# LuoweiZhou/VLP

Hardware: NVIDIA H100
Metric: image_text_samples_per_sec (higher is better)
Workload: dtype bf16

## Files before the change

### vlp_b200/csrc/common.cuh

```cuda
#pragma once
#include <cuda.h>
#include <cuda_bf16.h>
#include <cuda_runtime.h>
#include <stdint.h>

#include "wgmma.cuh"

namespace vlpk {

__device__ __forceinline__ uint32_t smem_u32(const void* p) {
  return static_cast<uint32_t>(__cvta_generic_to_shared(p));
}

__device__ __forceinline__ uint32_t lane_id() { return threadIdx.x & 31u; }

__device__ __forceinline__ bool elect_one() {
  uint32_t pred = 0;
  asm volatile(
      "{\n\t"
      ".reg .pred P;\n\t"
      "elect.sync _|P, 0xffffffff;\n\t"
      "selp.u32 %0, 1, 0, P;\n\t"
      "}\n"
      : "=r"(pred));
  return pred != 0;
}

__device__ __forceinline__ void mbar_init(uint64_t* bar, uint32_t count) {
  asm volatile("mbarrier.init.shared::cta.b64 [%0], %1;" ::"r"(smem_u32(bar)), "r"(count) : "memory");
}
__device__ __forceinline__ void fence_mbar_init() {
  asm volatile("fence.mbarrier_init.release.cluster;" ::: "memory");
}
__device__ __forceinline__ void fence_proxy_async_smem() {
  asm volatile("fence.proxy.async.shared::cta;" ::: "memory");
}
__device__ __forceinline__ void mbar_arrive_expect_tx(uint64_t* bar, uint32_t bytes) {
  asm volatile("mbarrier.arrive.expect_tx.shared::cta.b64 _, [%0], %1;" ::"r"(smem_u32(bar)), "r"(bytes)
               : "memory");
}
__device__ __forceinline__ void mbar_arrive(uint64_t* bar) {
  asm volatile("mbarrier.arrive.shared::cta.b64 _, [%0];" ::"r"(smem_u32(bar)) : "memory");
}
__device__ __forceinline__ bool mbar_try_wait(uint64_t* bar, uint32_t parity) {
  uint32_t ok;
  asm volatile(
      "{\n\t"
      ".reg .pred P;\n\t"
      "mbarrier.try_wait.parity.shared::cta.b64 P, [%1], %2;\n\t"
      "selp.u32 %0, 1, 0, P;\n\t"
      "}\n"
      : "=r"(ok)
      : "r"(smem_u32(bar)), "r"(parity)
      : "memory");
  return ok != 0;
}
__device__ __forceinline__ void mbar_wait(uint64_t* bar, uint32_t parity) {
  uint32_t spins = 0;
  while (!mbar_try_wait(bar, parity)) {
    if (++spins > (1u << 28)) { __trap(); }
  }
}

__device__ __forceinline__ void pdl_launch_dependents() { asm volatile("griddepcontrol.launch_dependents;" ::: "memory"); }
__device__ __forceinline__ void pdl_wait() { asm volatile("griddepcontrol.wait;" ::: "memory"); }

__device__ __forceinline__ void tma_prefetch_desc(const CUtensorMap* m) {
  asm volatile("prefetch.tensormap [%0];" ::"l"(reinterpret_cast<uint64_t>(m)) : "memory");
}
__device__ __forceinline__ void tma_load_2d(void* dst, const CUtensorMap* m, uint64_t* bar, int c0, int c1) {
  asm volatile(
      "cp.async.bulk.tensor.2d.shared::cluster.global.tile.mbarrier::complete_tx::bytes [%0], [%1, {%3, %4}], [%2];"
      ::"r"(smem_u32(dst)), "l"(reinterpret_cast<uint64_t>(m)), "r"(smem_u32(bar)), "r"(c0), "r"(c1)
      : "memory");
}
__device__ __forceinline__ void tma_load_3d(void* dst, const CUtensorMap* m, uint64_t* bar, int c0, int c1,
                                            int c2) {
  asm volatile(
      "cp.async.bulk.tensor.3d.shared::cluster.global.tile.mbarrier::complete_tx::bytes [%0], [%1, {%3, %4, %5}], "
      "[%2];" ::"r"(smem_u32(dst)),
      "l"(reinterpret_cast<uint64_t>(m)), "r"(smem_u32(bar)), "r"(c0), "r"(c1), "r"(c2)
      : "memory");
}
__device__ __forceinline__ void tma_store_2d(const CUtensorMap* m, const void* src, int c0, int c1) {
  asm volatile("cp.async.bulk.tensor.2d.global.shared::cta.tile.bulk_group [%0, {%2, %3}], [%1];" ::"l"(
                   reinterpret_cast<uint64_t>(m)),
               "r"(smem_u32(src)), "r"(c0), "r"(c1)
               : "memory");
}
__device__ __forceinline__ void tma_store_3d(const CUtensorMap* m, const void* src, int c0, int c1, int c2) {
  asm volatile("cp.async.bulk.tensor.3d.global.shared::cta.tile.bulk_group [%0, {%2, %3, %4}], [%1];" ::"l"(
                   reinterpret_cast<uint64_t>(m)),
               "r"(smem_u32(src)), "r"(c0), "r"(c1), "r"(c2)
               : "memory");
}
__device__ __forceinline__ void tma_reduce_add_2d(const CUtensorMap* m, const void* src, int c0, int c1) {
  asm volatile("cp.reduce.async.bulk.tensor.2d.global.shared::cta.add.tile.bulk_group [%0, {%2, %3}], [%1];" ::"l"(
                   reinterpret_cast<uint64_t>(m)),
               "r"(smem_u32(src)), "r"(c0), "r"(c1)
               : "memory");
}
__device__ __forceinline__ void tma_reduce_add_3d(const CUtensorMap* m, const void* src, int c0, int c1, int c2) {
  asm volatile("cp.reduce.async.bulk.tensor.3d.global.shared::cta.add.tile.bulk_group [%0, {%2, %3, %4}], [%1];" ::"l"(
                   reinterpret_cast<uint64_t>(m)),
               "r"(smem_u32(src)), "r"(c0), "r"(c1), "r"(c2)
               : "memory");
}
__device__ __forceinline__ void tma_store_commit() { asm volatile("cp.async.bulk.commit_group;" ::: "memory"); }
template <int N>
__device__ __forceinline__ void tma_store_wait_read() {
  asm volatile("cp.async.bulk.wait_group.read %0;" ::"n"(N) : "memory");
}
template <int N>
__device__ __forceinline__ void tma_store_wait() {
  asm volatile("cp.async.bulk.wait_group %0;" ::"n"(N) : "memory");
}

__device__ __forceinline__ void wgmma_fence() { asm volatile("wgmma.fence.sync.aligned;" ::: "memory"); }
__device__ __forceinline__ void wgmma_commit() { asm volatile("wgmma.commit_group.sync.aligned;" ::: "memory"); }
template <int N>
__device__ __forceinline__ void wgmma_wait() {
  asm volatile("wgmma.wait_group.sync.aligned %0;" ::"n"(N) : "memory");
}
template <int N>
__device__ __forceinline__ void reg_fence(float (&d)[N]) {
#pragma unroll
  for (int i = 0; i < N; ++i) asm volatile("" : "+f"(d[i])::"memory");
}

__device__ __forceinline__ uint64_t wgmma_desc_sw128(uint32_t saddr, uint32_t lbo_bytes, uint32_t sbo_bytes) {
  uint64_t d = 0;
  d |= static_cast<uint64_t>((saddr & 0x3FFFFu) >> 4);
  d |= static_cast<uint64_t>((lbo_bytes >> 4) & 0x3FFFu) << 16;
  d |= static_cast<uint64_t>((sbo_bytes >> 4) & 0x3FFFu) << 32;
  d |= 1ull << 62;
  return d;
}

__device__ __forceinline__ uint32_t pack_bf16x2(float lo, float hi) {
  __nv_bfloat162 v = __floats2bfloat162_rn(lo, hi);
  return *reinterpret_cast<uint32_t*>(&v);
}
__device__ __forceinline__ float2 unpack_bf16x2(uint32_t u) {
  __nv_bfloat162 v = *reinterpret_cast<__nv_bfloat162*>(&u);
  return __bfloat1622float2(v);
}
__device__ __forceinline__ float bf16_round(float x) { return __bfloat162float(__float2bfloat16_rn(x)); }

__device__ __forceinline__ float fast_ex2(float x) {
  float y;
  asm("ex2.approx.ftz.f32 %0, %1;" : "=f"(y) : "f"(x));
  return y;
}
__device__ __forceinline__ float fast_rcp(float x) {
  float y;
  asm("rcp.approx.ftz.f32 %0, %1;" : "=f"(y) : "f"(x));
  return y;
}

__device__ __forceinline__ void gelu_and_grad(float x, float& g, float& d) {
  const float ax = fabsf(x);
  const float e = fast_ex2(-0.72134752044448170f * x * x);
  const float t = fast_rcp(fmaf(0.3275911f * 0.70710678118654752f, ax, 1.0f));
  float poly = fmaf(1.061405429f, t, -1.453152027f);
  poly = fmaf(poly, t, 1.421413741f);
  poly = fmaf(poly, t, -0.284496736f);
  poly = fmaf(poly, t, 0.254829592f);
  poly *= t;
  const float erf_abs = fmaf(-poly, e, 1.0f);
  const float cdf = 0.5f * (1.0f + copysignf(erf_abs, x));
  g = x * cdf;
  d = fmaf(x * 0.3989422804014327f, e, cdf);
}

struct Philox {
  __device__ __forceinline__ static uint4 gen(uint64_t seed, uint64_t ctr_hi, uint64_t ctr_lo) {
    uint32_t k0 = static_cast<uint32_t>(seed), k1 = static_cast<uint32_t>(seed >> 32);
    uint4 c = make_uint4(static_cast<uint32_t>(ctr_lo), static_cast<uint32_t>(ctr_lo >> 32),
                         static_cast<uint32_t>(ctr_hi), static_cast<uint32_t>(ctr_hi >> 32));
#pragma unroll
    for (int i = 0; i < 10; ++i) {
      const uint32_t hi0 = __umulhi(0xD2511F53u, c.x), lo0 = 0xD2511F53u * c.x;
      const uint32_t hi1 = __umulhi(0xCD9E8D57u, c.z), lo1 = 0xCD9E8D57u * c.z;
      c = make_uint4(hi1 ^ c.y ^ k0, lo1, hi0 ^ c.w ^ k1, lo0);
      k0 += 0x9E3779B9u;
      k1 += 0xBB67AE85u;
    }
    return c;
  }
};
__device__ __forceinline__ uint32_t dropout_keep8(uint64_t seed, uint64_t site, uint64_t idx8, uint32_t thresh16) {
  const uint4 r = Philox::gen(seed, site, idx8);
  uint32_t m = 0;
  m |= ((r.x & 0xFFFFu) >= thresh16) ? 1u : 0u;
  m |= ((r.x >> 16) >= thresh16) ? 2u : 0u;
  m |= ((r.y & 0xFFFFu) >= thresh16) ? 4u : 0u;
  m |= ((r.y >> 16) >= thresh16) ? 8u : 0u;
  m |= ((r.z & 0xFFFFu) >= thresh16) ? 16u : 0u;
  m |= ((r.z >> 16) >= thresh16) ? 32u : 0u;
  m |= ((r.w & 0xFFFFu) >= thresh16) ? 64u : 0u;
  m |= ((r.w >> 16) >= thresh16) ? 128u : 0u;
  return m;
}

struct DropoutCfg {
  float p;
  float scale;
  uint32_t thresh16;
  uint64_t seed;
  uint64_t site;
  const unsigned long long* seed_ptr;
  const unsigned char* bits;
};

__device__ __forceinline__ uint64_t drop_seed(const DropoutCfg& d) {
  return (d.p > 0.f && d.seed_ptr != nullptr) ? d.seed + *d.seed_ptr : d.seed;
}

__host__ inline DropoutCfg make_dropout(float p, uint64_t seed, uint64_t site,
                                        const unsigned long long* seed_ptr = nullptr) {
  DropoutCfg d;
  d.bits = nullptr;
  d.seed_ptr = seed_ptr;
  d.p = p;
  d.scale = p > 0.f ? 1.0f / (1.0f - p) : 1.0f;
  d.thresh16 = static_cast<uint32_t>(p * 65536.0f);
  d.seed = seed;
  d.site = site;
  return d;
}

}
```

### vlp_b200/csrc/gemm.cu

```cuda
#include "gemm.cuh"

#include <cstdlib>

#include "host.cuh"

namespace vlpk {

static constexpr int BM = 128;
static constexpr int BK = 64;
static constexpr int NUM_THREADS = 288;
static constexpr int STG_BYTES = 64 * 128;
static constexpr int SMEM_MAX = 232448;
static constexpr int BN = 128;

struct GemmTmaps {
  CUtensorMap a;
  CUtensorMap b[3];
  CUtensorMap d0;
  CUtensorMap d1;
};

struct GemmArgs {
  int M, N, K;
  int b_seg_rows;
  int splits;
  int split_slices;
  const __nv_bfloat16* bias[3];
  const __nv_bfloat16* aux;
  long long ld_aux;
  float relu_scale;
  DropoutCfg drop;
  float* colsum;
};

template <int STAGES>
struct SmemLayout {
  static constexpr int A_BYTES = BM * BK * 2;
  static constexpr int B_BYTES = BN * BK * 2;
  static constexpr int STAGE_BYTES = A_BYTES + B_BYTES;
  static constexpr int OFF_STG = STAGES * STAGE_BYTES;
  static constexpr int OFF_BAR = OFF_STG + 4 * STG_BYTES;
  static constexpr int NUM_BARS = 2 * STAGES;
  static constexpr int TOTAL = OFF_BAR + NUM_BARS * 8;
  static constexpr int DYN_BYTES = TOTAL + 1024;
  static_assert(DYN_BYTES <= SMEM_MAX, "shared memory budget exceeded");
};

struct StageCount {
  static constexpr int value = (SMEM_MAX - 1024 - 4 * STG_BYTES - 256) / (BM * BK * 2 + BN * BK * 2);
};

__device__ __forceinline__ void wg_bar_sync(int cw) {
  asm volatile("bar.sync %0, 128;" ::"r"(cw + 1) : "memory");
}

template <bool A_MN, bool B_MN, int EPI>
__global__ void __launch_bounds__(NUM_THREADS, 1)
gemm_kernel(const __grid_constant__ GemmTmaps tm, const GemmArgs args) {
  constexpr int STAGES = StageCount::value;
  using L = SmemLayout<STAGES>;
  extern __shared__ uint8_t smem_raw[];
  uint8_t* smem = reinterpret_cast<uint8_t*>((reinterpret_cast<uintptr_t>(smem_raw) + 1023) & ~uintptr_t(1023));

  uint64_t* bars = reinterpret_cast<uint64_t*>(smem + L::OFF_BAR);
  uint64_t* full_bar = bars;
  uint64_t* empty_bar = bars + STAGES;

  pdl_launch_dependents();
  const int wg = threadIdx.x >> 7;
  const int lane = threadIdx.x & 31;

  const int num_m = (args.M + BM - 1) / BM;
  const int num_n = (args.N + BN - 1) / BN;
  const int total_kb = (args.K + BK - 1) / BK;
  const int kb_per = (total_kb + args.splits - 1) / args.splits;
  const int num_work = num_m * num_n * args.splits;

  if (threadIdx.x == 0) {
    tma_prefetch_desc(&tm.a);
    tma_prefetch_desc(&tm.b[0]);
    tma_prefetch_desc(&tm.d0);
    for (int i = 0; i < STAGES; ++i) {
      mbar_init(&full_bar[i], 1);
      mbar_init(&empty_bar[i], 8);
    }
    fence_mbar_init();
  }
  __syncthreads();
  pdl_wait();

  if (wg == 2) {
    {
      int stage = 0;
      uint32_t phase = 0;
      for (int w = blockIdx.x; w < num_work; w += gridDim.x) {
        const int n_blk = w % num_n;
        const int m_blk = (w / num_n) % num_m;
        const int split = w / (num_n * num_m);
        const int kb0 = split * kb_per;
        const int kb1 = min(total_kb, kb0 + kb_per);
        const int m0 = m_blk * BM;
        for (int kb = kb0; kb < kb1; ++kb) {
          mbar_wait(&empty_bar[stage], phase ^ 1u);
          if (elect_one()) {
            uint8_t* sA = smem + stage * L::STAGE_BYTES;
            uint8_t* sB = sA + L::A_BYTES;
            mbar_arrive_expect_tx(&full_bar[stage], L::STAGE_BYTES);
            if (!A_MN) {
              tma_load_2d(sA, &tm.a, &full_bar[stage], kb * BK, m0);
            } else {
#pragma unroll
              for (int j = 0; j < BM / 64; ++j) tma_load_2d(sA + j * 8192, &tm.a, &full_bar[stage], m0 + j * 64, kb * BK);
            }
            if (!B_MN) {
              const int n0 = n_blk * BN;
              const int seg = n0 / args.b_seg_rows;
              tma_load_2d(sB, &tm.b[seg], &full_bar[stage], kb * BK, n0 - seg * args.b_seg_rows);
            } else {
              const int k0 = kb * BK;
              const int seg = k0 / args.b_seg_rows;
#pragma unroll
              for (int j = 0; j < BN / 64; ++j)
                tma_load_2d(sB + j * 8192, &tm.b[seg], &full_bar[stage], n_blk * BN + j * 64, k0 - seg * args.b_seg_rows);
            }
          }
          __syncwarp();
          if (++stage == STAGES) {
            stage = 0;
            phase ^= 1u;
          }
        }
      }
    }
  } else {
    const int cw = wg;
    const int t = threadIdx.x - 128 * wg;
    const int fr = (t >> 5) * 16 + (lane >> 2);
    const int fc = (lane & 3) * 2;
    const bool store_thread = (t == 0);
    const uint64_t dseed = drop_seed(args.drop);
    constexpr bool HAS_BIAS = !B_MN && (EPI == EPI_STORE || EPI == EPI_GELU || EPI == EPI_RELU);
    uint8_t* stg0 = smem + L::OFF_STG + cw * 2 * STG_BYTES;
    uint8_t* stg1 = stg0 + STG_BYTES;
    const uint32_t a_base = smem_u32(smem) + cw * 8192;
    const uint32_t b_base = smem_u32(smem) + L::A_BYTES;
    int stage = 0;
    uint32_t phase = 0;
    uint32_t box_seq = 0;
    float acc[BN / 2];
    for (int w = blockIdx.x; w < num_work; w += gridDim.x) {
      const int n_blk = w % num_n;
      const int m_blk = (w / num_n) % num_m;
      const int split = w / (num_n * num_m);
      const int kb0 = split * kb_per;
      const int kb1 = min(total_kb, kb0 + kb_per);
      const int n0 = n_blk * BN;
      const int m0 = m_blk * BM + cw * 64;

      for (int kb = kb0; kb < kb1; ++kb) {
        mbar_wait(&full_bar[stage], phase);
        const uint32_t sa = a_base + stage * L::STAGE_BYTES;
        const uint32_t sb = b_base + stage * L::STAGE_BYTES;
        reg_fence(acc);
        wgmma_fence();
#pragma unroll
        for (int k = 0; k < BK / 16; ++k) {
          const uint64_t adesc = A_MN ? wgmma_desc_sw128(sa + k * 2048, 8192, 1024) : wgmma_desc_sw128(sa + k * 32, 16, 1024);
          const uint64_t bdesc = B_MN ? wgmma_desc_sw128(sb + k * 2048, 8192, 1024) : wgmma_desc_sw128(sb + k * 32, 16, 1024);
          wgmma_m64n128k16_ss<A_MN ? 1 : 0, B_MN ? 1 : 0>(acc, adesc, bdesc, (kb > kb0 || k > 0) ? 1u : 0u);
        }
        wgmma_commit();
        wgmma_wait<0>();
        reg_fence(acc);
        if (lane == 0) mbar_arrive(&empty_bar[stage]);
        if (++stage == STAGES) {
          stage = 0;
          phase ^= 1u;
        }
      }

      if (EPI == EPI_REDUCE_F32) {
        constexpr int NBOX = BN / 32;
#pragma unroll
        for (int c = 0; c < NBOX; ++c) {
          uint8_t* stg = (box_seq & 1u) ? stg1 : stg0;
          if (store_thread) tma_store_wait_read<1>();
          wg_bar_sync(cw);
#pragma unroll
          for (int j = 0; j < 8; ++j) {
            const int i = c * 16 + 2 * j;
            const int r = fr + 8 * (j & 1), col = 8 * (j >> 1) + fc;
            *reinterpret_cast<float2*>(stg + r * 128 + (((col >> 2) ^ (r & 7)) << 4) + (col & 3) * 4) = make_float2(acc[i], acc[i + 1]);
          }
          fence_proxy_async_smem();
          wg_bar_sync(cw);
          if (store_thread) {
            tma_reduce_add_3d(&tm.d0, stg, n0 + c * 32, m0, args.split_slices ? split : 0);
            tma_store_commit();
          }
          ++box_seq;
        }
      } else {
        constexpr int NBOX = BN / 64;
        const __nv_bfloat16* bp = nullptr;
        int bias_off = 0;
        if (HAS_BIAS) {
          const int seg = n0 / args.b_seg_rows;
          bp = args.bias[seg];
          bias_off = seg * args.b_seg_rows;
        }
#pragma unroll
        for (int c = 0; c < NBOX; ++c) {
          uint8_t* stg = (EPI == EPI_GELU) ? stg0 : ((box_seq & 1u) ? stg1 : stg0);
          if (store_thread) {
            if (EPI == EPI_GELU) tma_store_wait_read<0>(); else tma_store_wait_read<1>();
          }
          wg_bar_sync(cw);
#pragma unroll
          for (int j = 0; j < 16; ++j) {
            const int i = c * 32 + 2 * j;
            const int r = fr + 8 * (j & 1), col = 8 * (j >> 1) + fc;
            const int n = n0 + c * 64 + col;
            const long long m = m0 + r;
            float v0 = acc[i], v1 = acc[i + 1];
            if (HAS_BIAS) {
              if (bp != nullptr && n < args.N) {
                const float2 bb = unpack_bf16x2(__ldg(reinterpret_cast<const unsigned int*>(bp + n - bias_off)));
                v0 += bb.x;
                v1 += bb.y;
              }
            }
            const int so = r * 128 + (((col >> 3) ^ (r & 7)) << 4) + (col & 7) * 2;
            if (EPI == EPI_GELU) {
              float g0, d0, g1, d1;
              gelu_and_grad(v0, g0, d0);
              gelu_and_grad(v1, g1, d1);
              *reinterpret_cast<uint32_t*>(stg0 + so) = pack_bf16x2(d0, d1);
              *reinterpret_cast<uint32_t*>(stg1 + so) = pack_bf16x2(g0, g1);
              continue;
            }
            if (EPI == EPI_RELU) {
              uint32_t keep = 0xFFu;
              if (args.drop.p > 0.f)
                keep = dropout_keep8(dseed, args.drop.site, (static_cast<uint64_t>(m) * args.N + (n - fc)) >> 3, args.drop.thresh16);
              v0 = fmaxf(v0, 0.f);
              v1 = fmaxf(v1, 0.f);
              v0 = ((keep >> fc) & 1u) ? v0 * args.drop.scale : 0.f;
              v1 = ((keep >> (fc + 1)) & 1u) ? v1 * args.drop.scale : 0.f;
            } else if (EPI == EPI_ADD || EPI == EPI_MUL || EPI == EPI_DRELU) {
              float2 x = make_float2(0.f, 0.f);
              if (m < args.M && n < args.N) x = unpack_bf16x2(__ldg(reinterpret_cast<const unsigned int*>(args.aux + m * args.ld_aux + n)));
              if (EPI == EPI_ADD) {
                v0 += x.x;
                v1 += x.y;
              } else if (EPI == EPI_MUL) {
                v0 *= x.x;
                v1 *= x.y;
              } else {
                v0 = x.x > 0.f ? v0 * args.relu_scale : 0.f;
                v1 = x.y > 0.f ? v1 * args.relu_scale : 0.f;
              }
            }
            *reinterpret_cast<uint32_t*>(stg + so) = pack_bf16x2(v0, v1);
          }
          fence_proxy_async_smem();
          wg_bar_sync(cw);
          if (store_thread) {
            tma_store_2d(&tm.d0, stg, n0 + c * 64, m0);
            if (EPI == EPI_GELU) tma_store_2d(&tm.d1, stg1, n0 + c * 64, m0);
            tma_store_commit();
          }
          if (EPI != EPI_GELU && args.colsum != nullptr) {
            const int col = t & 63, r0 = (t >> 6) * 32;
            float acc_c = 0.f;
#pragma unroll 8
            for (int rr = r0; rr < r0 + 32; ++rr) {
              const __nv_bfloat16 v = *reinterpret_cast<const __nv_bfloat16*>(stg + rr * 128 + (((col >> 3) ^ (rr & 7)) << 4) + (col & 7) * 2);
              acc_c += __bfloat162float(v);
            }
            if (n0 + c * 64 + col < args.N) atomicAdd(args.colsum + n0 + c * 64 + col, acc_c);
          }
          ++box_seq;
        }
      }
    }
    if (store_thread) tma_store_wait<0>();
  }
}

template <bool A_MN, bool B_MN, int EPI>
static int launch_inst(const GemmTmaps& tm, const GemmArgs& args, int num_work, cudaStream_t stream) {
  constexpr int STAGES = StageCount::value;
  using L = SmemLayout<STAGES>;
  auto kfn = gemm_kernel<A_MN, B_MN, EPI>;
  static bool attr_set = false;
  if (!attr_set) {
    VLPK_CUDA(cudaFuncSetAttribute(kfn, cudaFuncAttributeMaxDynamicSharedMemorySize, L::DYN_BYTES));
    attr_set = true;
  }
  const int max_ctas = gemm_sms();
  const int ctas = num_work < max_ctas ? num_work : max_ctas;
  LaunchScope scope(A_MN ? CAT_GEMM_WGRAD : (B_MN ? CAT_GEMM_DGRAD : CAT_GEMM_FWD), 2.0 * args.M * args.N * args.K, stream);
  VLPK_CUDA(launch_ex(kfn, dim3(ctas), dim3(NUM_THREADS), L::DYN_BYTES, stream, 1, tm, args));
  return 0;
}

static int dispatch(const GemmDesc& g, const GemmTmaps& tm, const GemmArgs& args, int num_work, cudaStream_t s) {
  if (!g.a_mn && !g.b_mn) {
    switch (g.epi) {
      case EPI_STORE: return launch_inst<false, false, EPI_STORE>(tm, args, num_work, s);
      case EPI_GELU: return launch_inst<false, false, EPI_GELU>(tm, args, num_work, s);
      case EPI_RELU: return launch_inst<false, false, EPI_RELU>(tm, args, num_work, s);
      default: break;
    }
  } else if (!g.a_mn && g.b_mn) {
    switch (g.epi) {
      case EPI_STORE: return launch_inst<false, true, EPI_STORE>(tm, args, num_work, s);
      case EPI_ADD: return launch_inst<false, true, EPI_ADD>(tm, args, num_work, s);
      case EPI_MUL: return launch_inst<false, true, EPI_MUL>(tm, args, num_work, s);
      case EPI_DRELU: return launch_inst<false, true, EPI_DRELU>(tm, args, num_work, s);
      case EPI_REDUCE_F32: return launch_inst<false, true, EPI_REDUCE_F32>(tm, args, num_work, s);
      default: break;
    }
  } else if (g.a_mn && g.b_mn) {
    if (g.epi == EPI_REDUCE_F32) return launch_inst<true, true, EPI_REDUCE_F32>(tm, args, num_work, s);
    if (g.epi == EPI_STORE) return launch_inst<true, true, EPI_STORE>(tm, args, num_work, s);
  }
  set_error("gemm: unsupported (a_mn=%d, b_mn=%d, epi=%d) combination", (int)g.a_mn, (int)g.b_mn, g.epi);
  return -1;
}

static double tile_cost(int M, int N, int total_kb, int splits, bool reduce) {
  const int num_m = (M + BM - 1) / BM;
  const int num_n = (N + BN - 1) / BN;
  const long long tiles = static_cast<long long>(num_m) * num_n * splits;
  const int slots = gemm_sms();
  const long long rounds = (tiles + slots - 1) / slots;
  const int kb_per = (total_kb + splits - 1) / splits;
  const double mainloop = kb_per * (128.0 + double(BN));
  const double epi = (reduce ? 3.0 : 1.5) * BN;
  return rounds * (mainloop + epi + 60.0);
}

int plan_gemm(const GemmDesc& g, int* bn_out, int* splits_out) {
  const int seg_rows = g.nseg > 1 ? g.b_seg_rows : (g.b_mn ? g.K : g.N);
  const int total_kb = (g.K + BK - 1) / BK;
  const bool reduce = (g.epi == EPI_REDUCE_F32);
  VLPK_CHECK_ARG(g.bn == 0 || g.bn == BN, "gemm: no valid tile configuration (bn=%d; tiles are %d wide)", g.bn, BN);
  VLPK_CHECK_ARG(g.nseg == 1 || seg_rows % (g.b_mn ? BK : BN) == 0, "gemm: segment rows %d not tile aligned", seg_rows);
  int splits = 1;
  if (reduce) {
    const int max_s = total_kb / 8 > 0 ? total_kb / 8 : 1;
    if (g.splits > 0) {
      splits = g.splits < max_s ? g.splits : max_s;
    } else {
      double best = 1e300;
      for (int s = 1; s <= max_s; ++s) {
        const double c = tile_cost(g.M, g.N, total_kb, s, reduce);
        if (c < best) {
          best = c;
          splits = s;
        }
      }
    }
  }
  if (splits > total_kb) splits = total_kb;
  {
    const int kb_per = (total_kb + splits - 1) / splits;
    splits = (total_kb + kb_per - 1) / kb_per;
  }
  *bn_out = BN;
  *splits_out = splits;
  return 0;
}

int launch_gemm(const GemmDesc& g, cudaStream_t stream) {
  VLPK_CHECK_ARG(g.M > 0 && g.N > 0 && g.K > 0, "gemm: empty problem M=%d N=%d K=%d", g.M, g.N, g.K);
  VLPK_CHECK_ARG(g.N % 8 == 0, "gemm: N=%d must be a multiple of 8", g.N);
  VLPK_CHECK_ARG(g.nseg >= 1 && g.nseg <= 3, "gemm: nseg=%d", g.nseg);
  const int seg_rows = g.nseg > 1 ? g.b_seg_rows : (g.b_mn ? g.K : g.N);
  const bool reduce = (g.epi == EPI_REDUCE_F32);
  VLPK_CHECK_ARG(g.splits <= 1 || reduce, "gemm: split-K needs EPI_REDUCE_F32");
  VLPK_CHECK_ARG(g.b_rows == 0 || (g.nseg == 1 && g.b_rows <= (g.b_mn ? g.K : g.N)), "gemm: b_rows=%d needs a single B segment", g.b_rows);

  int bn = BN, splits = 1;
  VLPK_TRY(plan_gemm(g, &bn, &splits));

  GemmTmaps tm;
  memset(&tm, 0, sizeof(tm));
  if (!g.a_mn) {
    VLPK_TRY(make_tmap_2d(&tm.a, TM_BF16, g.A, g.K, g.M, g.lda, BK, BM));
  } else {
    VLPK_TRY(make_tmap_2d(&tm.a, TM_BF16, g.A, g.M, g.K, g.lda, 64, BK));
  }
  for (int s = 0; s < g.nseg; ++s) {
    if (!g.b_mn) {
      const int rows = g.nseg > 1 ? seg_rows : (g.b_rows > 0 ? g.b_rows : g.N);
      VLPK_TRY(make_tmap_2d(&tm.b[s], TM_BF16, g.B[s], g.K, rows, g.ldb, BK, bn));
    } else {
      const int rows = g.nseg > 1 ? seg_rows : (g.b_rows > 0 ? g.b_rows : g.K);
      VLPK_TRY(make_tmap_2d(&tm.b[s], TM_BF16, g.B[s], g.N, rows, g.ldb, 64, BK));
    }
  }
  for (int s = g.nseg; s < 3; ++s) tm.b[s] = tm.b[0];
  if (reduce) {
    VLPK_CHECK_ARG(g.split_stride == 0 || (g.split_stride % 4 == 0 && g.split_stride >= static_cast<int64_t>(g.M) * g.ldd0),
                   "gemm: split_stride %lld must be a multiple of 4 and cover M x ldd0", (long long)g.split_stride);
    const uint64_t dims[3] = {static_cast<uint64_t>(g.N), static_cast<uint64_t>(g.M), static_cast<uint64_t>(g.split_stride ? splits : 1)};
    const uint64_t strides[2] = {static_cast<uint64_t>(g.ldd0) * 4,
                                 static_cast<uint64_t>(g.split_stride ? g.split_stride : static_cast<int64_t>(g.M) * g.ldd0) * 4};
    const uint32_t box[3] = {32, 64, 1};
    VLPK_TRY(make_tmap(&tm.d0, TM_F32, 3, g.D0, dims, strides, box));
    tm.d1 = tm.d0;
  } else {
    VLPK_TRY(make_tmap_2d(&tm.d0, TM_BF16, g.D0, g.N, g.M, g.ldd0, 64, 64));
    if (g.epi == EPI_GELU) {
      VLPK_CHECK_ARG(g.D1 != nullptr, "gemm: EPI_GELU needs D1");
      VLPK_TRY(make_tmap_2d(&tm.d1, TM_BF16, g.D1, g.N, g.M, g.ldd1, 64, 64));
    } else {
      tm.d1 = tm.d0;
    }
  }
  VLPK_CHECK_ARG(g.colsum == nullptr || (!reduce && g.epi != EPI_GELU), "gemm: colsum fusion is for single-output bf16 epilogues");
  if (g.epi == EPI_ADD || g.epi == EPI_MUL || g.epi == EPI_DRELU) {
    VLPK_CHECK_ARG(g.aux != nullptr && (g.ld_aux % 8) == 0 && (reinterpret_cast<uintptr_t>(g.aux) & 15u) == 0,
                   "gemm: aux must be 16-byte aligned with ld %% 8 == 0");
  }

  GemmArgs a;
  a.M = g.M;
  a.N = g.N;
  a.K = g.K;
  a.b_seg_rows = seg_rows;
  a.splits = splits;
  a.split_slices = (reduce && g.split_stride > 0) ? 1 : 0;
  for (int s = 0; s < 3; ++s) a.bias[s] = (s < g.nseg) ? g.bias[s] : nullptr;
  a.aux = g.aux;
  a.ld_aux = g.ld_aux;
  a.relu_scale = g.relu_scale;
  a.colsum = g.colsum;
  a.drop = g.drop;

  const int num_m = (g.M + BM - 1) / BM;
  const int num_n = (g.N + bn - 1) / bn;
  const int num_work = num_m * num_n * splits;
  return dispatch(g, tm, a, num_work, stream);
}

}
```

Baseline: 3954.

## Ping-pong consumer warpgroups over whole tiles with register reallocation and async wgmma

Result: faster. 4167 (median of 6 runs) (+5.4%).

```diff
diff --git a/vlp_b200/csrc/common.cuh b/vlp_b200/csrc/common.cuh
--- a/vlp_b200/csrc/common.cuh
+++ b/vlp_b200/csrc/common.cuh
@@ -61,6 +61,12 @@
     if (++spins > (1u << 28)) { __trap(); }
   }
 }
+__device__ __forceinline__ void mbar_wait_flag(uint64_t* bar, uint32_t parity, bool& timed_out) {
+  uint32_t spins = 0;
+  while (!timed_out && !mbar_try_wait(bar, parity)) {
+    if (++spins > (1u << 28)) timed_out = true;
+  }
+}
 
 __device__ __forceinline__ void pdl_launch_dependents() { asm volatile("griddepcontrol.launch_dependents;" ::: "memory"); }
 __device__ __forceinline__ void pdl_wait() { asm volatile("griddepcontrol.wait;" ::: "memory"); }
@@ -122,6 +128,10 @@
 __device__ __forceinline__ void wgmma_wait() {
   asm volatile("wgmma.wait_group.sync.aligned %0;" ::"n"(N) : "memory");
 }
+template <uint32_t N>
+__device__ __forceinline__ void setmaxnreg_dec() { asm volatile("setmaxnreg.dec.sync.aligned.u32 %0;" ::"n"(N)); }
+template <uint32_t N>
+__device__ __forceinline__ void setmaxnreg_inc() { asm volatile("setmaxnreg.inc.sync.aligned.u32 %0;" ::"n"(N)); }
 template <int N>
 __device__ __forceinline__ void reg_fence(float (&d)[N]) {
 #pragma unroll
diff --git a/vlp_b200/csrc/gemm.cu b/vlp_b200/csrc/gemm.cu
--- a/vlp_b200/csrc/gemm.cu
+++ b/vlp_b200/csrc/gemm.cu
@@ -8,8 +8,11 @@
 
 static constexpr int BM = 128;
 static constexpr int BK = 64;
-static constexpr int NUM_THREADS = 288;
+static constexpr int NUM_THREADS = 384;
+static constexpr int PRODUCER_REGS = 24;
+static constexpr int CONSUMER_REGS = 240;
 static constexpr int STG_BYTES = 64 * 128;
+static constexpr int STG_PER_CONSUMER = 4;
 static constexpr int SMEM_MAX = 232448;
 static constexpr int BN = 128;
 
@@ -39,15 +42,15 @@
   static constexpr int B_BYTES = BN * BK * 2;
   static constexpr int STAGE_BYTES = A_BYTES + B_BYTES;
   static constexpr int OFF_STG = STAGES * STAGE_BYTES;
-  static constexpr int OFF_BAR = OFF_STG + 4 * STG_BYTES;
-  static constexpr int NUM_BARS = 2 * STAGES;
+  static constexpr int OFF_BAR = OFF_STG + 2 * STG_PER_CONSUMER * STG_BYTES;
+  static constexpr int NUM_BARS = 3 * STAGES;
   static constexpr int TOTAL = OFF_BAR + NUM_BARS * 8;
   static constexpr int DYN_BYTES = TOTAL + 1024;
   static_assert(DYN_BYTES <= SMEM_MAX, "shared memory budget exceeded");
 };
 
 struct StageCount {
-  static constexpr int value = (SMEM_MAX - 1024 - 4 * STG_BYTES - 256) / (BM * BK * 2 + BN * BK * 2);
+  static constexpr int value = (SMEM_MAX - 1024 - 2 * STG_PER_CONSUMER * STG_BYTES - 256) / (BM * BK * 2 + BN * BK * 2);
 };
 
 __device__ __forceinline__ void wg_bar_sync(int cw) {
@@ -64,10 +67,10 @@
 
   uint64_t* bars = reinterpret_cast<uint64_t*>(smem + L::OFF_BAR);
   uint64_t* full_bar = bars;
-  uint64_t* empty_bar = bars + STAGES;
+  uint64_t* empty_bar = bars + 2 * STAGES;
 
   pdl_launch_dependents();
-  const int wg = threadIdx.x >> 7;
+  const int wg = __shfl_sync(0xffffffffu, threadIdx.x >> 7, 0);
   const int lane = threadIdx.x & 31;
 
   const int num_m = (args.M + BM - 1) / BM;
@@ -80,20 +83,21 @@
     tma_prefetch_desc(&tm.a);
     tma_prefetch_desc(&tm.b[0]);
     tma_prefetch_desc(&tm.d0);
-    for (int i = 0; i < STAGES; ++i) {
-      mbar_init(&full_bar[i], 1);
-      mbar_init(&empty_bar[i], 8);
-    }
+    for (int i = 0; i < 2 * STAGES; ++i) mbar_init(&full_bar[i], 1);
+    for (int i = 0; i < STAGES; ++i) mbar_init(&empty_bar[i], 4);
     fence_mbar_init();
   }
   __syncthreads();
   pdl_wait();
 
-  if (wg == 2) {
-    {
+  if (wg == 0) {
+    setmaxnreg_dec<PRODUCER_REGS>();
+    if (threadIdx.x < 32) {
       int stage = 0;
       uint32_t phase = 0;
-      for (int w = blockIdx.x; w < num_work; w += gridDim.x) {
+      int item = 0;
+      for (int w = blockIdx.x; w < num_work; w += gridDim.x, ++item) {
+        uint64_t* fb = full_bar + (item & 1) * STAGES;
         const int n_blk = w % num_n;
         const int m_blk = (w / num_n) % num_m;
         const int split = w / (num_n * num_m);
@@ -105,23 +109,23 @@
           if (elect_one()) {
             uint8_t* sA = smem + stage * L::STAGE_BYTES;
             uint8_t* sB = sA + L::A_BYTES;
-            mbar_arrive_expect_tx(&full_bar[stage], L::STAGE_BYTES);
+            mbar_arrive_expect_tx(&fb[stage], L::STAGE_BYTES);
             if (!A_MN) {
-              tma_load_2d(sA, &tm.a, &full_bar[stage], kb * BK, m0);
+              tma_load_2d(sA, &tm.a, &fb[stage], kb * BK, m0);
             } else {
 #pragma unroll
-              for (int j = 0; j < BM / 64; ++j) tma_load_2d(sA + j * 8192, &tm.a, &full_bar[stage], m0 + j * 64, kb * BK);
+              for (int j = 0; j < BM / 64; ++j) tma_load_2d(sA + j * 8192, &tm.a, &fb[stage], m0 + j * 64, kb * BK);
             }
             if (!B_MN) {
               const int n0 = n_blk * BN;
               const int seg = n0 / args.b_seg_rows;
-              tma_load_2d(sB, &tm.b[seg], &full_bar[stage], kb * BK, n0 - seg * args.b_seg_rows);
+              tma_load_2d(sB, &tm.b[seg], &fb[stage], kb * BK, n0 - seg * args.b_seg_rows);
             } else {
               const int k0 = kb * BK;
               const int seg = k0 / args.b_seg_rows;
 #pragma unroll
               for (int j = 0; j < BN / 64; ++j)
-                tma_load_2d(sB + j * 8192, &tm.b[seg], &full_bar[stage], n_blk * BN + j * 64, k0 - seg * args.b_seg_rows);
+                tma_load_2d(sB + j * 8192, &tm.b[seg], &fb[stage], n_blk * BN + j * 64, k0 - seg * args.b_seg_rows);
             }
           }
           __syncwarp();
@@ -133,72 +137,95 @@
       }
     }
   } else {
-    const int cw = wg;
+    setmaxnreg_inc<CONSUMER_REGS>();
+    const int cw = wg - 1;
     const int t = threadIdx.x - 128 * wg;
     const int fr = (t >> 5) * 16 + (lane >> 2);
     const int fc = (lane & 3) * 2;
     const bool store_thread = (t == 0);
     const uint64_t dseed = drop_seed(args.drop);
     constexpr bool HAS_BIAS = !B_MN && (EPI == EPI_STORE || EPI == EPI_GELU || EPI == EPI_RELU);
-    uint8_t* stg0 = smem + L::OFF_STG + cw * 2 * STG_BYTES;
-    uint8_t* stg1 = stg0 + STG_BYTES;
-    const uint32_t a_base = smem_u32(smem) + cw * 8192;
+    uint8_t* stg_base = smem + L::OFF_STG + cw * STG_PER_CONSUMER * STG_BYTES;
+    const uint32_t a_base = smem_u32(smem);
     const uint32_t b_base = smem_u32(smem) + L::A_BYTES;
+    uint64_t* fb = full_bar + cw * STAGES;
     int stage = 0;
-    uint32_t phase = 0;
+    uint32_t phases = 0;
     uint32_t box_seq = 0;
-    float acc[BN / 2];
-    for (int w = blockIdx.x; w < num_work; w += gridDim.x) {
+    bool timed_out = false;
+    float acc[2][BN / 2];
+#pragma unroll
+    for (int i = 0; i < BN / 2; ++i) acc[0][i] = acc[1][i] = 0.f;
+    for (int w = blockIdx.x + cw * gridDim.x; w < num_work; w += 2 * gridDim.x) {
+      const int w_other = w - static_cast<int>(gridDim.x);
+      if (w_other >= static_cast<int>(blockIdx.x)) {
+        const int split_o = w_other / (num_n * num_m);
+        const int kb0_o = split_o * kb_per;
+        stage = (stage + min(total_kb, kb0_o + kb_per) - kb0_o) % STAGES;
+      }
       const int n_blk = w % num_n;
       const int m_blk = (w / num_n) % num_m;
       const int split = w / (num_n * num_m);
       const int kb0 = split * kb_per;
       const int kb1 = min(total_kb, kb0 + kb_per);
       const int n0 = n_blk * BN;
-      const int m0 = m_blk * BM + cw * 64;
-
+
+      int prev_stage = 0;
       for (int kb = kb0; kb < kb1; ++kb) {
-        mbar_wait(&full_bar[stage], phase);
+        mbar_wait_flag(&fb[stage], (phases >> stage) & 1u, timed_out);
+        phases ^= 1u << stage;
         const uint32_t sa = a_base + stage * L::STAGE_BYTES;
         const uint32_t sb = b_base + stage * L::STAGE_BYTES;
-        reg_fence(acc);
+        reg_fence(acc[0]);
+        reg_fence(acc[1]);
         wgmma_fence();
 #pragma unroll
         for (int k = 0; k < BK / 16; ++k) {
-          const uint64_t adesc = A_MN ? wgmma_desc_sw128(sa + k * 2048, 8192, 1024) : wgmma_desc_sw128(sa + k * 32, 16, 1024);
           const uint64_t bdesc = B_MN ? wgmma_desc_sw128(sb + k * 2048, 8192, 1024) : wgmma_desc_sw128(sb + k * 32, 16, 1024);
-          wgmma_m64n128k16_ss<A_MN ? 1 : 0, B_MN ? 1 : 0>(acc, adesc, bdesc, (kb > kb0 || k > 0) ? 1u : 0u);
+#pragma unroll
+          for (int h = 0; h < 2; ++h) {
+            const uint32_t sah = sa + h * 8192;
+            const uint64_t adesc = A_MN ? wgmma_desc_sw128(sah + k * 2048, 8192, 1024) : wgmma_desc_sw128(sah + k * 32, 16, 1024);
+            wgmma_m64n128k16_ss<A_MN ? 1 : 0, B_MN ? 1 : 0>(acc[h], adesc, bdesc, (kb > kb0 || k > 0) ? 1u : 0u);
+          }
         }
         wgmma_commit();
-        wgmma_wait<0>();
-        reg_fence(acc);
-        if (lane == 0) mbar_arrive(&empty_bar[stage]);
-        if (++stage == STAGES) {
-          stage = 0;
-          phase ^= 1u;
-        }
+        wgmma_wait<1>();
+        reg_fence(acc[0]);
+        reg_fence(acc[1]);
+        if (kb > kb0 && lane == 0) mbar_arrive(&empty_bar[prev_stage]);
+        prev_stage = stage;
+        if (++stage == STAGES) stage = 0;
       }
+      wgmma_wait<0>();
+      reg_fence(acc[0]);
+      reg_fence(acc[1]);
+      if (lane == 0) mbar_arrive(&empty_bar[prev_stage]);
 
       if (EPI == EPI_REDUCE_F32) {
         constexpr int NBOX = BN / 32;
 #pragma unroll
-        for (int c = 0; c < NBOX; ++c) {
-          uint8_t* stg = (box_seq & 1u) ? stg1 : stg0;
-          if (store_thread) tma_store_wait_read<1>();
-          wg_bar_sync(cw);
-#pragma unroll
-          for (int j = 0; j < 8; ++j) {
-            const int i = c * 16 + 2 * j;
-            const int r = fr + 8 * (j & 1), col = 8 * (j >> 1) + fc;
-            *reinterpret_cast<float2*>(stg + r * 128 + (((col >> 2) ^ (r & 7)) << 4) + (col & 3) * 4) = make_float2(acc[i], acc[i + 1]);
+        for (int h = 0; h < 2; ++h) {
+          const int m0 = m_blk * BM + h * 64;
+#pragma unroll
+          for (int c = 0; c < NBOX; ++c) {
+            uint8_t* stg = stg_base + (box_seq % STG_PER_CONSUMER) * STG_BYTES;
+            if (store_thread) tma_store_wait_read<STG_PER_CONSUMER - 1>();
+            wg_bar_sync(cw);
+#pragma unroll
+            for (int j = 0; j < 8; ++j) {
+              const int i = c * 16 + 2 * j;
+              const int r = fr + 8 * (j & 1), col = 8 * (j >> 1) + fc;
+              *reinterpret_cast<float2*>(stg + r * 128 + (((col >> 2) ^ (r & 7)) << 4) + (col & 3) * 4) = make_float2(acc[h][i], acc[h][i + 1]);
+            }
+            fence_proxy_async_smem();
+            wg_bar_sync(cw);
+            if (store_thread) {
+              tma_reduce_add_3d(&tm.d0, stg, n0 + c * 32, m0, args.split_slices ? split : 0);
+              tma_store_commit();
+            }
+            ++box_seq;
           }
-          fence_proxy_async_smem();
-          wg_bar_sync(cw);
-          if (store_thread) {
-            tma_reduce_add_3d(&tm.d0, stg, n0 + c * 32, m0, args.split_slices ? split : 0);
-            tma_store_commit();
-          }
-          ++box_seq;
         }
       } else {
         constexpr int NBOX = BN / 64;
@@ -210,81 +237,91 @@
           bias_off = seg * args.b_seg_rows;
         }
 #pragma unroll
-        for (int c = 0; c < NBOX; ++c) {
-          uint8_t* stg = (EPI == EPI_GELU) ? stg0 : ((box_seq & 1u) ? stg1 : stg0);
-          if (store_thread) {
-            if (EPI == EPI_GELU) tma_store_wait_read<0>(); else tma_store_wait_read<1>();
+        for (int h = 0; h < 2; ++h) {
+          const int m0 = m_blk * BM + h * 64;
+          int nh = n0;
+          const __nv_bfloat16* bph = bp;
+          uint64_t dsh = dseed;
+          asm volatile("" : "+r"(nh), "+l"(bph), "+l"(dsh));
+#pragma unroll
+          for (int c = 0; c < NBOX; ++c) {
+            uint8_t* stg = (EPI == EPI_GELU) ? stg_base + (box_seq & 1u) * 2 * STG_BYTES : stg_base + (box_seq % STG_PER_CONSUMER) * STG_BYTES;
+            uint8_t* stg_g = stg + STG_BYTES;
+            if (store_thread) {
+              if (EPI == EPI_GELU) tma_store_wait_read<STG_PER_CONSUMER / 2 - 1>(); else tma_store_wait_read<STG_PER_CONSUMER - 1>();
+            }
+            wg_bar_sync(cw);
+#pragma unroll
+            for (int j = 0; j < 16; ++j) {
+              const int i = c * 32 + 2 * j;
+              const int r = fr + 8 * (j & 1), col = 8 * (j >> 1) + fc;
+              const int n = nh + c * 64 + col;
+              const long long m = m0 + r;
+              float v0 = acc[h][i], v1 = acc[h][i + 1];
+              if (HAS_BIAS) {
+                if (bph != nullptr && n < args.N) {
+                  const float2 bb = unpack_bf16x2(__ldg(reinterpret_cast<const unsigned int*>(bph + n - bias_off)));
+                  v0 += bb.x;
+                  v1 += bb.y;
+                }
+              }
+              const int so = r * 128 + (((col >> 3) ^ (r & 7)) << 4) + (col & 7) * 2;
+              if (EPI == EPI_GELU) {
+                float g0, d0, g1, d1;
+                gelu_and_grad(v0, g0, d0);
+                gelu_and_grad(v1, g1, d1);
+                *reinterpret_cast<uint32_t*>(stg + so) = pack_bf16x2(d0, d1);
+                *reinterpret_cast<uint32_t*>(stg_g + so) = pack_bf16x2(g0, g1);
+                continue;
+              }
+              if (EPI == EPI_RELU) {
+                uint32_t keep = 0xFFu;
+                if (args.drop.p > 0.f)
+                  keep = dropout_keep8(dsh, args.drop.site, (static_cast<uint64_t>(m) * args.N + (n - fc)) >> 3, args.drop.thresh16);
+                v0 = fmaxf(v0, 0.f);
+                v1 = fmaxf(v1, 0.f);
+                v0 = ((keep >> fc) & 1u) ? v0 * args.drop.scale : 0.f;
+                v1 = ((keep >> (fc + 1)) & 1u) ? v1 * args.drop.scale : 0.f;
+              } else if (EPI == EPI_ADD || EPI == EPI_MUL || EPI == EPI_DRELU) {
+                float2 x = make_float2(0.f, 0.f);
+                if (m < args.M && n < args.N) x = unpack_bf16x2(__ldg(reinterpret_cast<const unsigned int*>(args.aux + m * args.ld_aux + n)));
+                if (EPI == EPI_ADD) {
+                  v0 += x.x;
+                  v1 += x.y;
+                } else if (EPI == EPI_MUL) {
+                  v0 *= x.x;
+                  v1 *= x.y;
+                } else {
+                  v0 = x.x > 0.f ? v0 * args.relu_scale : 0.f;
+                  v1 = x.y > 0.f ? v1 * args.relu_scale : 0.f;
+                }
+              }
+              *reinterpret_cast<uint32_t*>(stg + so) = pack_bf16x2(v0, v1);
+            }
+            fence_proxy_async_smem();
+            wg_bar_sync(cw);
+            if (store_thread) {
+              tma_store_2d(&tm.d0, stg, nh + c * 64, m0);
+              if (EPI == EPI_GELU) tma_store_2d(&tm.d1, stg_g, nh + c * 64, m0);
+              tma_store_commit();
+            }
+            if (EPI != EPI_GELU && args.colsum != nullptr) {
+              const int col = t & 63, r0 = (t >> 6) * 32;
+              float acc_c = 0.f;
+#pragma unroll 8
+              for (int rr = r0; rr < r0 + 32; ++rr) {
+                const __nv_bfloat16 v = *reinterpret_cast<const __nv_bfloat16*>(stg + rr * 128 + (((col >> 3) ^ (rr & 7)) << 4) + (col & 7) * 2);
+                acc_c += __bfloat162float(v);
+              }
+              if (nh + c * 64 + col < args.N) atomicAdd(args.colsum + nh + c * 64 + col, acc_c);
+            }
+            ++box_seq;
           }
-          wg_bar_sync(cw);
-#pragma unroll
-          for (int j = 0; j < 16; ++j) {
-            const int i = c * 32 + 2 * j;
-            const int r = fr + 8 * (j & 1), col = 8 * (j >> 1) + fc;
-            const int n = n0 + c * 64 + col;
-            const long long m = m0 + r;
-            float v0 = acc[i], v1 = acc[i + 1];
-            if (HAS_BIAS) {
-              if (bp != nullptr && n < args.N) {
-                const float2 bb = unpack_bf16x2(__ldg(reinterpret_cast<const unsigned int*>(bp + n - bias_off)));
-                v0 += bb.x;
-                v1 += bb.y;
-              }
-            }
-            const int so = r * 128 + (((col >> 3) ^ (r & 7)) << 4) + (col & 7) * 2;
-            if (EPI == EPI_GELU) {
-              float g0, d0, g1, d1;
-              gelu_and_grad(v0, g0, d0);
-              gelu_and_grad(v1, g1, d1);
-              *reinterpret_cast<uint32_t*>(stg0 + so) = pack_bf16x2(d0, d1);
-              *reinterpret_cast<uint32_t*>(stg1 + so) = pack_bf16x2(g0, g1);
-              continue;
-            }
-            if (EPI == EPI_RELU) {
-              uint32_t keep = 0xFFu;
-              if (args.drop.p > 0.f)
-                keep = dropout_keep8(dseed, args.drop.site, (static_cast<uint64_t>(m) * args.N + (n - fc)) >> 3, args.drop.thresh16);
-              v0 = fmaxf(v0, 0.f);
-              v1 = fmaxf(v1, 0.f);
-              v0 = ((keep >> fc) & 1u) ? v0 * args.drop.scale : 0.f;
-              v1 = ((keep >> (fc + 1)) & 1u) ? v1 * args.drop.scale : 0.f;
-            } else if (EPI == EPI_ADD || EPI == EPI_MUL || EPI == EPI_DRELU) {
-              float2 x = make_float2(0.f, 0.f);
-              if (m < args.M && n < args.N) x = unpack_bf16x2(__ldg(reinterpret_cast<const unsigned int*>(args.aux + m * args.ld_aux + n)));
-              if (EPI == EPI_ADD) {
-                v0 += x.x;
-                v1 += x.y;
-              } else if (EPI == EPI_MUL) {
-                v0 *= x.x;
-                v1 *= x.y;
-              } else {
-                v0 = x.x > 0.f ? v0 * args.relu_scale : 0.f;
-                v1 = x.y > 0.f ? v1 * args.relu_scale : 0.f;
-              }
-            }
-            *reinterpret_cast<uint32_t*>(stg + so) = pack_bf16x2(v0, v1);
-          }
-          fence_proxy_async_smem();
-          wg_bar_sync(cw);
-          if (store_thread) {
-            tma_store_2d(&tm.d0, stg, n0 + c * 64, m0);
-            if (EPI == EPI_GELU) tma_store_2d(&tm.d1, stg1, n0 + c * 64, m0);
-            tma_store_commit();
-          }
-          if (EPI != EPI_GELU && args.colsum != nullptr) {
-            const int col = t & 63, r0 = (t >> 6) * 32;
-            float acc_c = 0.f;
-#pragma unroll 8
-            for (int rr = r0; rr < r0 + 32; ++rr) {
-              const __nv_bfloat16 v = *reinterpret_cast<const __nv_bfloat16*>(stg + rr * 128 + (((col >> 3) ^ (rr & 7)) << 4) + (col & 7) * 2);
-              acc_c += __bfloat162float(v);
-            }
-            if (n0 + c * 64 + col < args.N) atomicAdd(args.colsum + n0 + c * 64 + col, acc_c);
-          }
-          ++box_seq;
         }
       }
     }
     if (store_thread) tma_store_wait<0>();
+    if (timed_out) __trap();
   }
 }
 
```
